# adrianalbert/domain-transfer-GAN

Measured on AMD Instinct MI355X. Metric: training images/sec, 256x256 Augmented CycleGAN step, 1/2/4/8 MI355X, higher is better.
Workload: dtype f32 tensors; conv products as 3 bf16 MFMAs on hi/lo-split fp32 operands (~2^-17 operand rounding), fp32 accumulate; parity vs the reference goldens: losses / single-pass images / cycle reconstructions <= 1e-3 on every fixture at step 0 (measured rec_A / rec_B <= 7.9e-4, profiles/r06_rec_errors.txt)

## Files before the change

### domain-transfer-gan_amd/_lib.py

```python
import ctypes
import os

_HERE = os.path.dirname(os.path.abspath(__file__))
LIB_PATH = os.environ.get("ACGAN_HIP_LIB") or os.path.join(_HERE, "libacgan_hip.so")

ACT_NONE, ACT_RELU, ACT_LRELU, ACT_TANH, ACT_SIGMOID = 0, 1, 2, 3, 4
PAD_ZERO, PAD_REFLECT = 0, 1
IMPL_MFMA, IMPL_DIRECT = 0, 1
PREC_F32, PREC_BF16, PREC_BF16X3 = 0, 1, 2
NLL_LAPLACE, NLL_GAUSSIAN = 0, 1

c_int, c_float, c_size_t, c_void_p = ctypes.c_int, ctypes.c_float, ctypes.c_size_t, ctypes.c_void_p


class ConvDesc(ctypes.Structure):
    _fields_ = [(k, c_int) for k in ("N", "Hi", "Wi", "Ci", "Ho", "Wo", "Co", "K", "stride", "pad", "pad_mode", "Cir", "Cor")]


class LatentMlpParams(ctypes.Structure):
    _fields_ = [("w", c_void_p * 4), ("b", c_void_p * 4), ("gamma", c_void_p * 3), ("beta", c_void_p * 3),
                ("run_mean", c_void_p * 3), ("run_var", c_void_p * 3), ("head_act", c_int)]


class LatentMlpGrads(ctypes.Structure):
    _fields_ = [("dw", c_void_p * 4), ("db", c_void_p * 4), ("dgamma", c_void_p * 3), ("dbeta", c_void_p * 3)]


class AdamGroup(ctypes.Structure):
    _fields_ = [("p", c_void_p), ("g", c_void_p), ("m", c_void_p), ("v", c_void_p), ("n", c_size_t), ("sumsq", c_void_p)]


class EmaGroup(ctypes.Structure):
    _fields_ = [("p", c_void_p), ("e", c_void_p), ("n", c_size_t)]


class PackItem(ctypes.Structure):
    _fields_ = [("w", c_void_p), ("wf", c_void_p), ("wb", c_void_p), ("Or", c_int), ("Ir", c_int), ("K", c_int), ("Ci", c_int), ("Co", c_int)]


MAX_SEGMENTS = 96


class Segments(ctypes.Structure):
    _fields_ = [("dst", c_void_p * MAX_SEGMENTS), ("off", c_int * MAX_SEGMENTS), ("len", c_int * MAX_SEGMENTS), ("n", c_int)]


class NormSumsDesc(ctypes.Structure):
    _fields_ = [("x", c_void_p), ("mean", c_void_p), ("rstd", c_void_p), ("gamma", c_void_p), ("beta", c_void_p),
                ("gstride", c_int), ("sign_mask", c_void_p), ("act", c_int), ("part", c_void_p)]


WINDOW_MAX = 64


class WindowPlan(ctypes.Structure):
    _fields_ = [(k, c_int) for k in ("H", "W", "S", "R", "ny", "nx")] + [("oy", c_int * WINDOW_MAX), ("ox", c_int * WINDOW_MAX)]


ADAM_MAX_GROUPS = 8
EMA_MAX_GROUPS = 8
_P = c_void_p
_D = ctypes.POINTER(ConvDesc)
_MP = ctypes.POINTER(LatentMlpParams)
_MG = ctypes.POINTER(LatentMlpGrads)

SIGNATURES = {
    "acg_version": (c_int, []),
    "acg_last_error": (ctypes.c_char_p, []),
    "acg_last_kernel": (ctypes.c_char_p, []),
    "acg_set_conv_impl": (c_int, [c_int]),
    "acg_set_conv_precision": (c_int, [c_int]),
    "acg_minmax_scale_nhwc_to_nchw": (c_int, [_P, _P, c_int, c_int, c_int, c_int, c_int, _P]),
    "acg_nchw_to_nhwc16": (c_int, [_P, _P, c_int, c_int, c_int, c_int, c_int, _P]),
    "acg_nhwc16_to_nchw": (c_int, [_P, _P, c_int, c_int, c_int, c_int, c_int, _P]),
    "acg_concat_channels": (c_int, [_P, c_int, c_int, _P, c_int, c_int, _P, c_int, c_size_t, _P]),
    "acg_split_channels": (c_int, [_P, c_int, _P, c_int, c_int, _P, c_int, c_int, c_size_t, _P]),
    "acg_ncols_pad": (c_int, [c_int]),
    "acg_packed_wf_elems": (c_size_t, [c_int, c_int, c_int]),
    "acg_packed_wb_elems": (c_size_t, [c_int, c_int, c_int]),
    "acg_pack_conv_weight": (c_int, [_P, c_int, c_int, c_int, c_int, c_int, _P, _P, _P]),
    "acg_pad_vector": (c_int, [_P, c_int, _P, c_int, _P]),
    "acg_conv2d_fwd": (c_int, [_D, _P, _P, _P, _P, c_int, _P]),
    "acg_conv2d_bwd_data_workspace_bytes": (c_size_t, [_D]),
    "acg_conv2d_bwd_data": (c_int, [_D, _P, _P, _P, _P, c_size_t, _P]),
    "acg_s16_encode": (c_int, [_P, _P, c_size_t, _P]),
    "acg_s16_decode": (c_int, [_P, _P, c_size_t, _P]),
    "acg_conv2d_s16_supported": (c_int, [_D]),
    "acg_conv2d_fwd_s16": (c_int, [_D, _P, _P, _P, _P, c_int, _P, c_int, _P]),
    "acg_conv2d_bwd_data_s16": (c_int, [_D, _P, _P, _P, _P, c_size_t, _P, _P, _P, c_int, _P]),
    "acg_conv2d_fwd_s16_mask": (c_int, [_D, _P, _P, _P, _P, _P, _P]),
    "acg_conv2d_bwd_data_s16_mask": (c_int, [_D, _P, _P, _P, _P, c_size_t, _P, _P]),
    "acg_conv2d_bwd_data_s16_sums_supported": (c_int, [_D]),
    "acg_conv2d_bwd_data_s16_sums": (c_int, [_D, _P, _P, _P, _P, c_size_t, _P, _P, ctypes.POINTER(NormSumsDesc), _P]),
    "acg_conv2d_bwd_data_sums_supported": (c_int, [_D]),
    "acg_conv2d_bwd_data_sums": (c_int, [_D, _P, _P, _P, _P, c_size_t, ctypes.POINTER(NormSumsDesc), _P]),
    "acg_conv2d_bwd_weight_s16": (c_int, [_D, _P, _P, _P, _P, c_int, c_int, _P, c_size_t, c_int, _P]),
    "acg_conv2d_bwd_weight_workspace_bytes": (c_size_t, [_D]),
    "acg_conv2d_bwd_weight": (c_int, [_D, _P, _P, _P, _P, c_int, c_int, _P, c_size_t, c_int, _P]),
    "acg_conv_transpose2d_fwd": (c_int, [_D, _P, _P, _P, _P, c_int, _P]),
    "acg_conv_transpose2d_fwd_stats_supported": (c_int, [_D]),
    "acg_conv_transpose2d_fwd_stats": (c_int, [_D, _P, _P, _P, _P, _P, _P]),
    "acg_conv_transpose2d_bwd_data": (c_int, [_D, _P, _P, _P, _P]),
    "acg_conv_transpose2d_bwd_weight": (c_int, [_D, _P, _P, _P, _P, c_int, c_int, _P, c_size_t, c_int, _P]),
    "acg_norm_workspace_bytes": (c_size_t, [c_int, c_size_t, c_int]),
    "acg_conv2d_fwd_stats_supported": (c_int, [_P]),
    "acg_conv2d_bwd_data_add_supported": (c_int, [_P]),
    "acg_conv2d_bwd_data_add": (c_int, [_P, _P, _P, _P, _P, _P, _P, c_size_t, _P]),
    "acg_pack_conv_weights_multi_supported": (c_int, [c_int, c_int, c_int]),
    "acg_pack_conv_weights_multi": (c_int, [_P, c_int, _P]),
    "acg_debug_mid_event": (c_int, [_P]),
    "acg_probe_mfma_rate": (c_int, [_P, c_size_t, c_int, ctypes.POINTER(ctypes.c_double), _P]),
    "acg_mask_apply": (c_int, [_P, _P, _P, c_size_t, _P]),
    "acg_dropout_apply": (c_int, [_P, _P, c_float, _P, c_size_t, _P]),
    "acg_conv2d_bwd_data_relu": (c_int, [_P, _P, _P, _P, _P, _P, c_size_t, _P]),
    "acg_conv2d_fwd_stats": (c_int, [_P, _P, _P, _P, _P, _P, _P]),
    "acg_norm_stats_from_partials": (c_int, [_P, c_int, c_size_t, c_int, c_int, c_float, c_int, _P, _P, _P]),
    "acg_norm_stats": (c_int, [_P, c_int, c_size_t, c_int, c_float, c_int, _P, _P, _P, _P, c_float, _P, c_size_t, _P]),
    "acg_bn_eval_stats": (c_int, [_P, _P, c_int, c_int, c_float, _P, _P, _P]),
    "acg_norm_apply": (c_int, [_P, _P, _P, _P, _P, c_int, _P, _P, _P, c_int, c_size_t, c_int, c_int, c_int, _P]),
    "acg_norm_bwd": (c_int, [_P, _P, _P, _P, _P, _P, _P, _P, c_int, _P, _P, _P, _P, c_int, c_int, c_int, c_size_t, c_int, c_int,
                             c_int, c_int, _P, c_size_t, _P]),
    "acg_norm_bwd_partials": (c_int, [_P, _P, _P, _P, _P, _P, _P, _P, c_int, _P, _P, _P, _P, c_int, c_int, c_int, c_size_t, c_int,
                                      c_int, c_int, c_int, _P, c_int, _P, c_size_t, _P]),
    "acg_norm_bwd_sums": (c_int, [_P, _P, _P, _P, _P, _P, c_int, c_size_t, c_int, c_int, _P, c_size_t, _P]),
    "acg_norm_bwd_apply": (c_int, [_P, _P, _P, _P, _P, _P, c_int, _P, _P, _P, c_int, c_size_t, c_size_t, c_int, c_int, c_int, _P]),
    "acg_act_bwd": (c_int, [_P, _P, _P, c_size_t, c_int, _P]),
    "acg_linear_fwd": (c_int, [_P, _P, _P, _P, c_int, c_int, c_int, c_int, c_int, c_int, _P]),
    "acg_linear_bwd": (c_int, [_P, _P, _P, _P, _P, _P, _P, c_int, c_int, c_int, c_int, c_int, c_int, _P]),
    "acg_latent_mlp_supported": (c_int, [c_int, c_int, c_int]),
    "acg_latent_mlp_fwd": (c_int, [_MP, _P, c_int, c_int, c_int, c_int, c_float, c_float, _P, _P, _P, _P]),
    "acg_latent_mlp_bwd": (c_int, [_MP, _MG, _P, c_int, c_int, c_int, c_int, _P, _P, _P, _P, _P, c_int, _P]),
    "acg_segments_accumulate": (c_int, [_P, ctypes.POINTER(Segments), c_int, _P]),
    "acg_spatial_mean_fwd": (c_int, [_P, _P, c_int, c_size_t, c_int, _P]),
    "acg_spatial_mean_bwd": (c_int, [_P, _P, c_int, c_size_t, c_int, _P]),
    "acg_reduce_workspace_bytes": (c_size_t, [c_size_t]),
    "acg_mse_const_fwd": (c_int, [_P, c_size_t, c_int, c_int, c_float, _P, _P, c_size_t, _P]),
    "acg_mse_const_bwd": (c_int, [_P, c_size_t, c_int, c_int, c_float, _P, _P, _P]),
    "acg_bce_const_fwd": (c_int, [_P, c_size_t, c_int, c_int, c_float, _P, _P, c_size_t, _P]),
    "acg_bce_const_bwd": (c_int, [_P, c_size_t, c_int, c_int, c_float, _P, _P, _P]),
    "acg_l1_fwd": (c_int, [_P, _P, c_size_t, c_int, c_int, _P, _P, c_size_t, _P]),
    "acg_l1_bwd": (c_int, [_P, _P, c_size_t, c_int, c_int, _P, _P, _P, _P]),
    "acg_mean_fwd": (c_int, [_P, c_size_t, c_int, c_int, _P, _P, c_size_t, _P]),
    "acg_sumsq": (c_int, [_P, c_size_t, _P, _P, c_size_t, _P]),
    "acg_pixel_nll_workspace_bytes": (c_size_t, [c_int, c_size_t]),
    "acg_pixel_nll_fwd": (c_int, [c_int, _P, _P, _P, c_int, c_size_t, c_int, c_int, _P, _P, c_size_t, _P]),
    "acg_pixel_nll_bwd": (c_int, [c_int, _P, _P, _P, c_int, c_size_t, c_int, c_int, _P, _P, _P, _P]),
    "acg_latent_bound_step": (c_int, [c_int, c_int, c_int, _P, _P, _P, _P, _P, _P, _P, c_float, c_float, c_float, _P, _P, _P,
                                      _P]),
    "acg_ensemble_workspace_bytes": (c_size_t, [c_int, c_size_t]),
    "acg_ensemble_stats": (c_int, [_P, _P, c_int, c_int, c_size_t, c_int, c_int, ctypes.POINTER(c_float), c_int, _P, _P, _P, _P,
                                   _P, _P, _P, c_size_t, _P]),
    "acg_radial_spectrum_workspace_bytes": (c_size_t, [c_int, c_int, c_int]),
# ... 88 lines not shown
```

### domain-transfer-gan_amd/csrc/conv_internal.h

```cpp
#pragma once
#include "common.h"

#define ACG_KC 16

struct Taps {
    int n;
    short dy[64];
    short dx[64];
    short w[64];
    int pk[64];
    int gpk[64];
    int ngrp;
};

static inline Taps acg_taps_pack(const Taps &t)
{
    Taps r = t;
    for (int i = 0; i < 64; ++i)
        r.pk[i] = i < t.n ? ((t.dy[i] & 0xff) | ((t.dx[i] & 0xff) << 8) | ((int)t.w[i] << 16)) : 0;
    return r;
}

struct Geom {
    int Hin, Win, Cin;
    int Hout, Wout, Cout;
    int GH, GW;
    int os, oy0, ox0;
    int is;
    int reflect;
    int act;
    int ncols_pad;
    long long w_elems;
    int fold_p = 0, fold_H = 0, fold_W = 0;
    float *out2 = nullptr;
    const float *addend = nullptr;
    const unsigned *addend_mask = nullptr;
    const float *relu_src = nullptr;
    int out_s16 = 0, relu_s16 = 0;
    unsigned *mask_out = nullptr;
    const unsigned *relu_mask = nullptr;
    int unpad = 0;
    const float *colfix = nullptr;
    const float *ns_x = nullptr, *ns_mean = nullptr, *ns_rstd = nullptr, *ns_gamma = nullptr, *ns_beta = nullptr;
    const unsigned *ns_mask = nullptr;
    float *ns_part = nullptr;
    int ns_gstride = 0, ns_act = 0;
    float *stats = nullptr;
    int stats_cpi = 0, stats_chunk0 = 0;
    int nphase = 0;
    int ph_ntaps = 0;
    int thin;
    int bk8;
    long long Mtot;
};

int acg_igemm_launch(const float *in, const float *wp, const float *bias, float *out, const Geom &g, const Taps &t,
                     hipStream_t st);

struct WGeom {
    int Hin, Win, Cin;
    int Hg, Wg, Cg;
    int is;
    int reflect;
    int CiP, CoP;
    int nsplit;
    long long Mtot;
    long long m_per_split;
    int thin;
    int bias_from;
    float *bias_part;
};
int acg_wgrad_launch(const float *x, const float *dy, float *part, const WGeom &g, const Taps &t, hipStream_t st);
void acg_wgrad_tiles(int Ci, int Co, int *bci, int *bco, int ntaps);
int acg_wgrad_taps_per_wg(int Ci, int Co, int ntaps, int thin);
bool acg_wgrad_krowg_shape_ok(int K, int stride, int pad, int reflect, int Wi, int Wo, int Cx, int Cg);
bool acg_wgrad_krowg_ok(const WGeom &g, const Taps &t);
int acg_wgrad_krowg_launch(const float *x, const float *dy, float *part, const WGeom &g, const Taps &t, hipStream_t st);

extern int g_acg_precision;
extern int g_acg_conv_impl;

static inline bool use_bf16() { return g_acg_precision != ACG_PREC_F32 && g_acg_conv_impl == ACG_IMPL_MFMA; }
static inline bool bf16x3_mfma() { return g_acg_precision == ACG_PREC_BF16X3 && g_acg_conv_impl == ACG_IMPL_MFMA; }
static inline bool thin_ok(int creal, int K) { return creal >= 1 && creal <= 4 && K > 1 && g_acg_conv_impl == ACG_IMPL_MFMA; }
static inline bool thin_in(const acg_conv_desc *d) { return thin_ok(d->Cir, d->K) && !thin_ok(d->Cor, d->K); }
static inline bool thin_out(const acg_conv_desc *d) { return thin_ok(d->Cor, d->K) && !thin_ok(d->Cir, d->K); }
static inline bool thin_valu_c(int C) { return !use_bf16() && (C == 16 || C == 32 || C == 64); }
__host__ __device__ static inline int c16(int c) { return (c + 15) / 16 * 16; }
__host__ __device__ static inline int wb_slabs(int K) { return K * K + (K == 3 ? 3 : 0); }
enum { ACG_TAIL_NONE = 0, ACG_TAIL_NPACK, ACG_TAIL_TROW };
static inline int pack_tail(int K, int Ck, int Cn)
{
    if (K <= 1 || K > 7) return ACG_TAIL_NONE;
    return c16(Cn) == 16 && c16(Ck) == 32 ? ACG_TAIL_NPACK : (c16(Ck) == 16 && c16(Cn) == 32 ? ACG_TAIL_TROW : ACG_TAIL_NONE);
}
static inline size_t pack_tail_elems(int tail, int K)
{
    return tail == ACG_TAIL_NPACK ? (size_t)K * (K + 3) * 512 : (tail == ACG_TAIL_TROW ? (size_t)K * 1024 : 0);
}
static inline size_t wf_regular_elems(int K, int Ci, int Co) { return (size_t)K * K * (c16(Ci) / 8) * acg_ncols_pad(c16(Co)) * 8; }
static inline size_t wb_regular_elems(int K, int Ci, int Co) { return (size_t)wb_slabs(K) * (c16(Co) / 8) * acg_ncols_pad(c16(Ci)) * 8; }
int acg_igemm_x3_ws_launch(const float *in, const void *wp, const float *bias, float *out, const Geom &g, const Taps &t,
                           long long n_w_elems, hipStream_t st, float *stats = nullptr);
bool acg_igemm_uses_ws(const Geom &g);
bool acg_igemm_x3_pre_ok(const Geom &g, const Taps &t);
int acg_igemm_x3_pre_launch(const void *in, const void *wp, const float *bias, float *out, const Geom &g, const Taps &t,
                            long long n_w_elems, hipStream_t st, float *stats = nullptr);
bool acg_conv_patch16_ok(const Geom &g, const Taps &t);
int acg_conv_patch16_launch(const float *in, const void *wp, const float *bias, float *out, const Geom &g, const Taps &t,
                            long long n_w_elems, hipStream_t st);
bool acg_conv_rows_ok(const Geom &g, const Taps &t);
int acg_conv_rows_launch(const float *in, const void *wp, const float *bias, float *out, const Geom &g, const Taps &t,
                         long long n_w_elems, hipStream_t st);
bool acg_conv_patchn_ok(const Geom &g, const Taps &t);
int acg_conv_patchn_launch(const float *in, const void *wn, const float *bias, float *out, const Geom &g, const Taps &t, hipStream_t st);
bool acg_conv_thinrow_ok(const Geom &g, const Taps &t);
int acg_conv_thinrow_launch(const float *in, const void *wr, const float *bias, float *out, const Geom &g, const Taps &t, hipStream_t st);
bool acg_igemm_ph4_ok(const Geom &g);
bool acg_ph4_plan(const Taps &t, const int nt[4], Taps *out);
int acg_igemm_ph4_launch(const float *in, const void *wp, const float *bias, float *out, const Geom &g, const Taps &plan,
                         long long n_w_elems, hipStream_t st);
int acg_igemm_bf16_launch(const float *in, const void *wp, const float *bias, float *out, const Geom &g, const Taps &t,
                          int bn, long long n_w_elems, hipStream_t st);
int acg_wgrad_bf16_launch(const float *x, const float *dy, float *part, const WGeom &g, const Taps &t, int bci, int bco,
                          hipStream_t st);
bool acg_wgrad_krow_shape_ok(int K, int stride, int pad, int Hi, int Wi, int Ho, int Wo, int Cx, int Cg);
bool acg_wgrad_krow_ok(const WGeom &g, const Taps &t);
int acg_wgrad_krow_launch(const float *x, const float *dy, float *part, const WGeom &g, hipStream_t st);
int acg_wgrad_krow_s16_launch(const void *x, const void *dy, float *part, const WGeom &g, hipStream_t st);
bool acg_wgrad_krow_s_shape_ok(int K, int stride, int pad, int Hi, int Wi, int Ho, int Wo, int Cx, int Cg);
bool acg_wgrad_krow_s_ok(const WGeom &g, const Taps &t);
bool acg_wgrad_thin_patch_shape_ok(int K, int stride, int Hthin, int Wthin, int Hwide, int Wwide, int Cthin, int Cwide);
bool acg_wgrad_thin_patch_ok(const WGeom &g, const Taps &t, int *K, int *flip);
int acg_wgrad_thin_patch_tiles(const WGeom &g);
int acg_wgrad_thin_patch_launch(const float *thin, const float *wide, float *part, const WGeom &g, const Taps &t, hipStream_t st);
int acg_wgrad_krow_s_launch(const float *x, const float *dy, float *part, const WGeom &g, hipStream_t st);

int acg_thin_out_launch(const float *in, const float *wn, const float *bias, float *out, const Geom &g, const Taps &t, hipStream_t st);
int acg_dgrad_colfix_launch(const acg_conv_desc *d, const void *dy, const float *wb, long long w_lo_elems, float *colfix, hipStream_t st);
int acg_reflect_fold_launch(const acg_conv_desc *d, const float *dxp, float *dx, hipStream_t st);
int acg_reflect_fold_frame_launch(const acg_conv_desc *d, const float *dxp, float *dx, const float *addend, const float *relu_src,
                                  const unsigned *addend_mask, int out_s16, int relu_s16, hipStream_t st);
size_t acg_colsum_ws_bytes(long long M, int C);
int acg_colsum_launch(const float *dy, long long M, int C, int Cr, float *db, float *ws, hipStream_t st, int accumulate);
int acg_wgrad_reduce_launch(const float *part, int nsplit, int KK, int CiP, int CoP, int Or, int Ir, float *dw, int thin,
                            int accumulate, const float *bias_part, int Cp, int Cr, float *db, int bias_slots, hipStream_t st);
int acg_direct_fwd_launch(const acg_conv_desc *d, const float *x, const float *wf, const float *bias, float *y, int act, hipStream_t st);
int acg_direct_dgrad_launch(const acg_conv_desc *d, const float *dy, const float *wb, const float *bias, float *dx, int act, hipStream_t st);
int acg_direct_wgrad_launch(const acg_conv_desc *d, const float *x, const float *dy, float *dw, int Or, int Ir, int accumulate, hipStream_t st);

#ifdef __HIPCC__
typedef unsigned acg_u32x4 __attribute__((ext_vector_type(4)));
__device__ __forceinline__ unsigned acg_masked_off(unsigned off, bool ok)
{
    const unsigned keep = 0u - (unsigned)ok;
    return (off & keep) | ~keep;
}
__device__ __forceinline__ void acg_split8(const float (&v)[8], acg_u32x4 &hi, acg_u32x4 &lo)
{
    typedef __bf16 bf16x2_t __attribute__((ext_vector_type(2)));
    typedef float f32x2_t __attribute__((ext_vector_type(2)));
#pragma unroll
    for (int q = 0; q < 4; ++q) {
        const unsigned h = __builtin_bit_cast(unsigned, __builtin_convertvector((f32x2_t){v[2 * q], v[2 * q + 1]}, bf16x2_t));
        const float ha = __builtin_bit_cast(float, h << 16), hb = __builtin_bit_cast(float, h & 0xffff0000u);
        hi[q] = h;
        lo[q] = __builtin_bit_cast(unsigned, __builtin_convertvector((f32x2_t){v[2 * q] - ha, v[2 * q + 1] - hb}, bf16x2_t));
    }
}
__device__ __forceinline__ acg_u32x4 acg_round8(const float (&v)[8])
{
    typedef __bf16 bf16x2_t __attribute__((ext_vector_type(2)));
    typedef float f32x2_t __attribute__((ext_vector_type(2)));
    acg_u32x4 r;
#pragma unroll
    for (int q = 0; q < 4; ++q)
        r[q] = __builtin_bit_cast(unsigned, __builtin_convertvector((f32x2_t){v[2 * q], v[2 * q + 1]}, bf16x2_t));
    return r;
}
#endif
```

### domain-transfer-gan_amd/csrc/conv_x3_pre.hip

```cpp
#include "common.h"
#include "conv_internal.h"
#include <cstdlib>
#include <type_traits>

typedef __bf16 bf16x8 __attribute__((ext_vector_type(8)));
typedef float f32x4 __attribute__((ext_vector_type(4)));
typedef unsigned u32x4 __attribute__((ext_vector_type(4)));

namespace {
constexpr int BM = 128, BN = 128, KC = 32, NK8 = KC / 8;
constexpr int BPL = BN * 8;
constexpr int B_IMG = NK8 * BPL;
__device__ __forceinline__ int lds_at(int plane, int row, int pl) { return plane * pl + ((row ^ (2 * plane)) * 8); }
constexpr int PROW = 80;
constexpr int PPIECES = 11;
constexpr int PIMG = PPIECES * 1024;
constexpr int ABUF = 2 * PIMG;
constexpr int A_BYTES = 2 * ABUF;
constexpr int BBUF = 2 * B_IMG * 2;
constexpr int LDS_BYTES = A_BYTES + 2 * BBUF;
constexpr int NPW = 6;
constexpr unsigned NO_PIX = 0xFFFFFFFFu;
}

// ... 457 lines not shown
                sq += dlt * dlt;
            }
        }
        __syncthreads();
        if (sw) redf[h * BN + c] = sq;
        __syncthreads();
        if (sw && h == 0 && n0 + c < g.Cout) {
            float *o = stats + ((m0 / BM) * 2) * g.Cout + n0 + c;
            o[0] = mu;
            o[g.Cout] = redf[c] + redf[BN + c];
        }
    }
    char *const base0 = (char *)out, *const base1 = (char *)g.out2;
    if (g.out_s16) {
        const char *rsrc = (const char *)g.relu_src;
        constexpr int NK = BM * (BN / 8) / ET;
        u32x4 sv[NK];
#pragma unroll
        for (int k = 0; k < NK; ++k) {
            const int idx = tid + ET * k, row = idx / (BN / 8), c8 = idx - row * (BN / 8);
            const unsigned po = pix_off[row];
            const bool live = po != NO_PIX && (po >> 31) && n0 + c8 * 8 < g.Cout;
            const size_t boff = (size_t)(po & 0x7fffffffu) * 16 + (size_t)(n0 + c8 * 8) * 4;
            if (g.relu_mask != nullptr) sv[k][0] = live ? g.relu_mask[boff >> 7] : 0u;
            else sv[k] = *(const u32x4 *)(rsrc != nullptr && live ? rsrc + boff : in);
        }
#pragma unroll
        for (int k = 0; k < NK; ++k) {
            const int idx = tid + ET * k, row = idx / (BN / 8), c8 = idx - row * (BN / 8);
            const unsigned po = pix_off[row];
            const bool live = po != NO_PIX && n0 + c8 * 8 < g.Cout;
            const size_t boff = (size_t)(po & 0x7fffffffu) * 16 + (size_t)(n0 + c8 * 8) * 4;
            const f32x4 t0 = *(const f32x4 *)&tile[row * TS + c8 * 8], t1 = *(const f32x4 *)&tile[row * TS + c8 * 8 + 4];
            float v[8] = {t0[0], t0[1], t0[2], t0[3], t1[0], t1[1], t1[2], t1[3]};
            if (g.relu_mask != nullptr && (po >> 31)) {
                const unsigned bits = sv[k][0] >> (8 * (c8 & 3));
#pragma unroll
                for (int q = 0; q < 8; ++q) v[q] = (bits >> q) & 1u ? v[q] : 0.f;
            } else if (rsrc != nullptr && (po >> 31)) {
#pragma unroll
                for (int q = 0; q < 4; ++q) {
                    const unsigned a = sv[k][q] & 0xffffu, b = sv[k][q] >> 16;
                    v[2 * q] = (a - 1u) < 0x7fffu ? v[2 * q] : 0.f;
                    v[2 * q + 1] = (b - 1u) < 0x7fffu ? v[2 * q + 1] : 0.f;
                }
            }
            if (g.mask_out != nullptr) {
                unsigned w = 0u;
#pragma unroll
                for (int q = 0; q < 8; ++q) w |= (v[q] > 0.f ? 1u : 0u) << q;
                w = live ? w << (8 * (c8 & 3)) : 0u;
                w |= __shfl_xor(w, 1);
                w |= __shfl_xor(w, 2);
                if (live && (c8 & 3) == 0) g.mask_out[boff >> 7] = w;
            }
            if (!live) continue;
            if (g.fold_p > 0 && !(po >> 31)) {
                *(f32x4 *)(base0 + boff) = t0;
                *(f32x4 *)(base0 + boff + 16) = t1;
                continue;
            }
            acg_u32x4 hi, lo;
            acg_split8(v, hi, lo);
            char *dst = ((po >> 31) ? base1 : base0) + boff;
            *(acg_u32x4 *)dst = hi;
            *(acg_u32x4 *)(dst + 16) = lo;
        }
        TILE_STAMP_END()
        return;
    }
    {
#pragma unroll 4
        for (int k = 0; k < BM * (BN / 4) / ET; ++k) {
            const int idx = tid + ET * k, row = idx / (BN / 4), c4 = idx - row * (BN / 4);
            const unsigned po = pix_off[row];
            if (po != NO_PIX && n0 + c4 * 4 < g.Cout)
                *(f32x4 *)(((po >> 31) ? base1 : base0) + (size_t)(po & 0x7fffffffu) * 16 + (size_t)(n0 + c4 * 4) * 4) = *(const f32x4 *)&tile[row * TS + c4 * 4];
        }
    }
    TILE_STAMP_END()
}
#undef TILE_STAMP_END

static bool pre_rowp(const Geom &g, const Taps &t, int *kdim, int *dxmin, int *kstep)
{
    if (g.is != 1 || g.os != 1 || g.oy0 != 0 || g.ox0 != 0 || g.Hout != g.GH || g.Wout != g.GW) return false;
    int k = 1;
    while (k * k < t.n) ++k;
    if (k * k != t.n || k < 2) return false;
    const int nseg_max = 2 + BM / g.GW, rows_max = BM + nseg_max * (k - 1);
    if (rows_max * 5 > PPIECES * 64 || (BM + (k - 1)) * 5 <= (PPIECES - 1) * 64) return false;
    int mn = t.dx[0];
    for (int i = 1; i < t.n; ++i) mn = t.dx[i] < mn ? t.dx[i] : mn;
    for (int i = 0; i < t.n; ++i)
        if (t.dy[i] != t.dy[(i / k) * k] || t.dx[i] < mn || t.dx[i] >= mn + k) return false;
    const int ks = t.dx[0] == mn ? 1 : -1;
    for (int i = 0; i < t.n; ++i)
        if (t.dx[i] != (ks > 0 ? mn + i % k : mn + k - 1 - i % k)) return false;
    *kdim = k; *dxmin = mn; *kstep = ks;
    return true;
}

bool acg_igemm_x3_pre_ok(const Geom &g, const Taps &t)
{
    int a, b, c;
    return g_acg_precision == ACG_PREC_BF16X3 && g_acg_conv_impl == ACG_IMPL_MFMA && !g.thin && g.Cout >= 128 && g.Cin % 32 == 0 &&
           pre_rowp(g, t, &a, &b, &c);
}

int acg_igemm_x3_pre_launch(const void *in, const void *wp, const float *bias, float *out, const Geom &g0, const Taps &t,
                            long long n_w_elems, hipStream_t st, float *stats)
{
    Geom g = g0;
    g.thin = 0;
    int kdim = 0, dxmin = 0, kstep = 1;
    ACG_REQUIRE(acg_igemm_x3_pre_ok(g, t) && pre_rowp(g, t, &kdim, &dxmin, &kstep), "igemm_conv_x3_pre: unsupported geometry");
    dim3 grid(acg_cdiv(g.Mtot, BM) * (g.ncols_pad / BN));
    const long long nimg = g.Mtot / ((long long)g.GH * g.GW);
    const long long in_bytes = nimg * g.Hin * g.Win * g.Cin * 4;
    const long long out_bytes = nimg * g.Hout * g.Wout * g.Cout * 4;
    const long long w_bytes = n_w_elems * 2 * 2;
    ACG_REQUIRE(in_bytes < (1LL << 32) && w_bytes < (1LL << 32) && out_bytes < (1LL << 34) && g.Mtot < (1LL << 30),
                "igemm_conv_x3_pre: operand exceeds the buffer-addressing limit");
    ACG_REQUIRE(stats == nullptr || (((long long)g.GH * g.GW) % BM == 0 && g.act == ACG_ACT_NONE && !g.out_s16),
                "igemm_conv_x3_pre: per-tile statistics need whole 128-pixel tiles per image, no activation, fp32 output");
    ACG_REQUIRE(!g.out_s16 || (g.addend == nullptr && g.Cout % 8 == 0), "igemm_conv_x3_pre: pre-split output takes no addend");
    ACG_REQUIRE(g.relu_src == nullptr || ((g.fold_p > 0 || g.unpad) && g.out_s16), "igemm_conv_x3_pre: the ReLU source needs the frame path and pre-split output");
    ACG_REQUIRE((g.mask_out == nullptr && g.relu_mask == nullptr) || (g.out_s16 && g.Cout % 32 == 0 && g.ncols_pad == g.Cout && g.fold_p == 0 &&
                                                                        (g.relu_mask == nullptr || (g.unpad && g.relu_src == nullptr))),
                "igemm_conv_x3_pre: sign bitmasks go with pre-split output, 32-multiple channels and the un-padded grid");
    ACG_REQUIRE((g.ns_part == nullptr && (g.addend == nullptr || g.out_s16)) || out_bytes < (1LL << 32),
                "igemm_conv_x3_pre: side inputs (skip addend / norm sums) on a tensor of 4 GiB or more");
    ACG_REQUIRE(g.ns_part == nullptr || (g.unpad && !g.out_s16 && g.Cout % 4 == 0 && (g.ns_act == ACG_ACT_NONE || g.ns_act == ACG_ACT_RELU) &&
                                       g.ns_x != nullptr && g.ns_mean != nullptr && g.ns_rstd != nullptr &&
                                       (g.ns_act == ACG_ACT_NONE || g.ns_mask != nullptr || (g.ns_gamma != nullptr && g.ns_beta != nullptr))),
                "igemm_conv_x3_pre: the norm sums ride on the un-padded fp32 data gradient (act NONE / RELU)");
    ACG_REQUIRE(!g.unpad || (g.GW % BM == 0 && g.GH >= 4 && kdim == 3 && !g.reflect && g.fold_p == 0 && g.out2 == out && g.act == ACG_ACT_NONE),
                "igemm_conv_x3_pre: the un-padded reflect data gradient needs whole-row tiles of a 3x3 layer");
    const unsigned inb = (unsigned)in_bytes, wb = (unsigned)w_bytes, wlo = (unsigned)(n_w_elems * 2);
    const Taps tp = acg_taps_pack(t);
#define X3_PRE(R, S, U) hipLaunchKernelGGL((igemm_conv_x3_pre<R, S, U>), grid, dim3(512), 0, st, (const char *)in, (const __bf16 *)wp, bias, out, g, tp, inb, wb, wlo, stats, kdim, dxmin, kstep)
    ACG_REQUIRE(g.ns_part == nullptr || (!g.reflect && stats == nullptr), "igemm_conv_x3_pre: norm sums on a forward launch");
    if (g.reflect) { if (stats) X3_PRE(true, true, false); else X3_PRE(true, false, false); }
    else if (g.ns_part != nullptr) X3_PRE(false, false, true);
    else { if (stats) X3_PRE(false, true, false); else X3_PRE(false, false, false); }
#undef X3_PRE
    ACG_CHECK_LAUNCH("igemm_conv_x3_pre");
    acg_note_kernel("igemm_conv_x3_pre<REFLECT=%d,STATS=%d%s>", g.reflect ? 1 : 0, stats ? 1 : 0, g.ns_part != nullptr ? ",SUMS=1" : "");
    return ACG_OK;
}
```

### include/acgan_hip.h

```cpp
#ifndef ACGAN_HIP_H
#define ACGAN_HIP_H

#include <stddef.h>
#include <stdint.h>

#ifdef __cplusplus
extern "C" {
#endif

#define ACG_VERSION 118

typedef enum {
    ACG_OK = 0,
    ACG_ERR_INVALID = -1,
    ACG_ERR_WORKSPACE = -2,
    ACG_ERR_LAUNCH = -3,
    ACG_ERR_COMM = -4
} acg_status;

typedef enum {
    ACG_ACT_NONE = 0, ACG_ACT_RELU = 1, ACG_ACT_LRELU = 2 , ACG_ACT_TANH = 3, ACG_ACT_SIGMOID = 4
} acg_act;
typedef enum { ACG_PAD_ZERO = 0, ACG_PAD_REFLECT = 1 } acg_pad_mode;
typedef enum { ACG_IMPL_MFMA = 0, ACG_IMPL_DIRECT = 1 } acg_conv_impl;
typedef enum { ACG_PREC_F32 = 0, ACG_PREC_BF16 = 1, ACG_PREC_BF16X3 = 2 } acg_precision;

typedef struct {
    int N, Hi, Wi, Ci;
    int Ho, Wo, Co;
    int K, stride, pad, pad_mode;
    int Cir, Cor;
} acg_conv_desc;

int acg_version(void);
const char *acg_last_error(void);
const char *acg_last_kernel(void);
int acg_debug_mid_event(void *event);
int acg_probe_mfma_rate(float *scratch, size_t scratch_floats, int iters, double *flops_out, void *stream);
int acg_set_conv_impl(int impl);
int acg_set_conv_precision(int prec);

int acg_minmax_scale_nhwc_to_nchw(const float *raw, float *out_nchw, int N, int H, int W, int Craw, int C, void *stream);

int acg_nchw_to_nhwc16(const float *src, float *dst, int N, int C, int H, int W, int Cp, void *stream);
int acg_nhwc16_to_nchw(const float *src, float *dst, int N, int C, int H, int W, int Cp, void *stream);
int acg_concat_channels(const float *a, int Ca, int Cap, const float *b, int Cb, int Cbp, float *dst, int Cdp,
                        size_t npix, void *stream);
int acg_split_channels(const float *gdst, int Cdp, float *ga, int Ca, int Cap, float *gb, int Cb, int Cbp,
                       size_t npix, void *stream);

int acg_ncols_pad(int c);
size_t acg_packed_wf_elems(int K, int Ci, int Co);
size_t acg_packed_wb_elems(int K, int Ci, int Co);
int acg_pack_conv_weight(const float *w_oihw, int Or, int Ir, int K, int Ci, int Co, float *wf, float *wb, void *stream);
typedef struct {
    const float *w;
    float *wf, *wb;
    int Or, Ir, K, Ci, Co;
} acg_pack_item;
int acg_pack_conv_weights_multi_supported(int Or, int Ir, int K);
int acg_pack_conv_weights_multi(const acg_pack_item *items, int n, void *stream);
int acg_pad_vector(const float *src, int n, float *dst, int np, void *stream);

int acg_conv2d_fwd(const acg_conv_desc *d, const float *x, const float *wf, const float *bias, float *y, int act,
                   void *stream);
int acg_conv2d_fwd_stats_supported(const acg_conv_desc *d);
int acg_conv2d_fwd_stats(const acg_conv_desc *d, const float *x, const float *wf, const float *bias, float *y,
                         float *stats, void *stream);
size_t acg_conv2d_bwd_data_workspace_bytes(const acg_conv_desc *d);
int acg_conv2d_bwd_data(const acg_conv_desc *d, const float *dy, const float *wb, float *dx, void *workspace,
                        size_t ws_bytes, void *stream);
int acg_conv2d_bwd_data_add_supported(const acg_conv_desc *d);
int acg_conv2d_bwd_data_add(const acg_conv_desc *d, const float *dy, const float *wb, const float *addend,
                            const unsigned *addend_sign_mask, float *dx, void *ws, size_t ws_bytes, void *stream);
int acg_conv2d_bwd_data_relu(const acg_conv_desc *d, const float *dy, const float *wb, const float *x, float *dx,
                             void *ws, size_t ws_bytes, void *stream);
int acg_s16_encode(const float *x, void *y_s16, size_t n, void *stream);
int acg_s16_decode(const void *x_s16, float *y, size_t n, void *stream);
int acg_conv2d_s16_supported(const acg_conv_desc *d);
int acg_conv2d_fwd_s16(const acg_conv_desc *d, const void *x_s16, const float *wf, const float *bias, void *y, int act,
                       float *stats, int out_s16, void *stream);
int acg_conv2d_bwd_data_s16(const acg_conv_desc *d, const void *dy_s16, const float *wb, void *dx, void *ws, size_t ws_bytes,
                            const float *addend, const unsigned *addend_sign_mask, const void *relu_src_s16, int out_s16,
                            void *stream);
typedef struct acg_norm_sums {
    const float *x, *mean, *rstd;
    const float *gamma, *beta;
    int gstride;
    const unsigned *sign_mask;
    int act;
    float *part;
} acg_norm_sums;
int acg_conv2d_bwd_data_s16_sums_supported(const acg_conv_desc *d);
int acg_conv2d_bwd_data_s16_sums(const acg_conv_desc *d, const void *dy_s16, const float *wb, float *dx, void *ws,
                                 size_t ws_bytes, const float *addend, const unsigned *addend_sign_mask,
                                 const acg_norm_sums *ns, void *stream);
int acg_conv2d_bwd_data_sums_supported(const acg_conv_desc *d);
int acg_conv2d_bwd_data_sums(const acg_conv_desc *d, const float *dy, const float *wb, float *dx, void *ws, size_t ws_bytes,
                             const acg_norm_sums *ns, void *stream);
int acg_conv2d_fwd_s16_mask(const acg_conv_desc *d, const void *x_s16, const float *wf, const float *bias, void *y_s16,
                            unsigned *sign_mask, void *stream);
int acg_conv2d_bwd_data_s16_mask(const acg_conv_desc *d, const void *dy_s16, const float *wb, void *dx_s16, void *ws,
                                 size_t ws_bytes, const unsigned *relu_sign_mask, void *stream);
int acg_conv2d_bwd_weight_s16(const acg_conv_desc *d, const void *x_s16, const void *dy_s16, float *dw, float *db, int Or,
                              int Ir, void *ws, size_t ws_bytes, int accumulate, void *stream);
size_t acg_conv2d_bwd_weight_workspace_bytes(const acg_conv_desc *d);
int acg_conv2d_bwd_weight(const acg_conv_desc *d, const float *x, const float *dy, float *dw_oihw, float *db,
                          int Or, int Ir, void *workspace, size_t ws_bytes, int accumulate, void *stream);

int acg_conv_transpose2d_fwd(const acg_conv_desc *d, const float *x, const float *wb, const float *bias, float *y,
                             int act, void *stream);
int acg_conv_transpose2d_fwd_stats_supported(const acg_conv_desc *d);
int acg_conv_transpose2d_fwd_stats(const acg_conv_desc *d, const float *x, const float *wb, const float *bias, float *y,
                                   float *stats, void *stream);
int acg_conv_transpose2d_bwd_data(const acg_conv_desc *d, const float *dy, const float *wf, float *dx, void *stream);
int acg_conv_transpose2d_bwd_weight(const acg_conv_desc *d, const float *x, const float *dy, float *dw_oihw,
                                    float *db, int Or, int Ir, void *workspace, size_t ws_bytes, int accumulate,
                                    void *stream);

// ... 191 lines not shown
```

Measured before the change: 222.4.

## Add 256-pixel tile bf16x3 conv kernel with dedicated DMA producer waves

Adds a new implicit-GEMM conv kernel for 3x3 reflect-padded layers with 128-multiple channels. It uses a 256x128 output tile, 768 threads (8 MFMA waves plus 4 producer waves issuing buffer-to-LDS loads), and 4-deep weight buffering. The aim is to raise weight and patch reuse per workgroup and to overlap the loads with the MFMA work. The existing 128-pixel kernel now dispatches to it when the geometry qualifies. The cost is a larger LDS footprint and lower occupancy (3 waves/EU), plus fewer workgroups on smaller layers, which could hurt load balance.

Measured after the change: 224.1, median of 6. About the same (+0.7%).

```diff
diff --git a/domain-transfer-gan_amd/_lib.py b/domain-transfer-gan_amd/_lib.py
--- a/domain-transfer-gan_amd/_lib.py
+++ b/domain-transfer-gan_amd/_lib.py
@@ -68,6 +68,7 @@
     "acg_version": (c_int, []),
     "acg_last_error": (ctypes.c_char_p, []),
     "acg_last_kernel": (ctypes.c_char_p, []),
+    "acg_last_x3_tile_pixels": (c_int, []),
     "acg_set_conv_impl": (c_int, [c_int]),
     "acg_set_conv_precision": (c_int, [c_int]),
     "acg_minmax_scale_nhwc_to_nchw": (c_int, [_P, _P, c_int, c_int, c_int, c_int, c_int, _P]),
diff --git a/domain-transfer-gan_amd/csrc/conv_internal.h b/domain-transfer-gan_amd/csrc/conv_internal.h
--- a/domain-transfer-gan_amd/csrc/conv_internal.h
+++ b/domain-transfer-gan_amd/csrc/conv_internal.h
@@ -106,6 +106,11 @@
 bool acg_igemm_x3_pre_ok(const Geom &g, const Taps &t);
 int acg_igemm_x3_pre_launch(const void *in, const void *wp, const float *bias, float *out, const Geom &g, const Taps &t,
                             long long n_w_elems, hipStream_t st, float *stats = nullptr);
+bool acg_x3_pre_rowp(const Geom &g, const Taps &t, int *kdim, int *dxmin, int *kstep);
+bool acg_igemm_x3_t256_ok(const Geom &g, const Taps &t);
+int acg_igemm_x3_t256_launch(const void *in, const void *wp, const float *bias, float *out, const Geom &g, const Taps &t,
+                             long long n_w_elems, hipStream_t st, float *stats);
+void acg_note_x3_tile(int pixels);
 bool acg_conv_patch16_ok(const Geom &g, const Taps &t);
 int acg_conv_patch16_launch(const float *in, const void *wp, const float *bias, float *out, const Geom &g, const Taps &t,
                             long long n_w_elems, hipStream_t st);
diff --git a/domain-transfer-gan_amd/csrc/conv_x3_pre.hip b/domain-transfer-gan_amd/csrc/conv_x3_pre.hip
--- a/domain-transfer-gan_amd/csrc/conv_x3_pre.hip
+++ b/domain-transfer-gan_amd/csrc/conv_x3_pre.hip
@@ -563,7 +563,7 @@
 }
 #undef TILE_STAMP_END
 
-static bool pre_rowp(const Geom &g, const Taps &t, int *kdim, int *dxmin, int *kstep)
+bool acg_x3_pre_rowp(const Geom &g, const Taps &t, int *kdim, int *dxmin, int *kstep)
 {
     if (g.is != 1 || g.os != 1 || g.oy0 != 0 || g.ox0 != 0 || g.Hout != g.GH || g.Wout != g.GW) return false;
     int k = 1;
@@ -586,7 +586,7 @@
 {
     int a, b, c;
     return g_acg_precision == ACG_PREC_BF16X3 && g_acg_conv_impl == ACG_IMPL_MFMA && !g.thin && g.Cout >= 128 && g.Cin % 32 == 0 &&
-           pre_rowp(g, t, &a, &b, &c);
+           acg_x3_pre_rowp(g, t, &a, &b, &c);
 }
 
 int acg_igemm_x3_pre_launch(const void *in, const void *wp, const float *bias, float *out, const Geom &g0, const Taps &t,
@@ -595,7 +595,12 @@
     Geom g = g0;
     g.thin = 0;
     int kdim = 0, dxmin = 0, kstep = 1;
-    ACG_REQUIRE(acg_igemm_x3_pre_ok(g, t) && pre_rowp(g, t, &kdim, &dxmin, &kstep), "igemm_conv_x3_pre: unsupported geometry");
+    ACG_REQUIRE(acg_igemm_x3_pre_ok(g, t) && acg_x3_pre_rowp(g, t, &kdim, &dxmin, &kstep), "igemm_conv_x3_pre: unsupported geometry");
+    if (acg_igemm_x3_t256_ok(g, t)) {
+        if (int rc = acg_igemm_x3_t256_launch(in, wp, bias, out, g, t, n_w_elems, st, stats)) return rc;
+        acg_note_kernel("igemm_conv_x3_pre<REFLECT=1,STATS=%d>", stats ? 1 : 0);
+        return ACG_OK;
+    }
     dim3 grid(acg_cdiv(g.Mtot, BM) * (g.ncols_pad / BN));
     const long long nimg = g.Mtot / ((long long)g.GH * g.GW);
     const long long in_bytes = nimg * g.Hin * g.Win * g.Cin * 4;
@@ -627,6 +632,7 @@
     else { if (stats) X3_PRE(false, true, false); else X3_PRE(false, false, false); }
 #undef X3_PRE
     ACG_CHECK_LAUNCH("igemm_conv_x3_pre");
+    acg_note_x3_tile(BM);
     acg_note_kernel("igemm_conv_x3_pre<REFLECT=%d,STATS=%d%s>", g.reflect ? 1 : 0, stats ? 1 : 0, g.ns_part != nullptr ? ",SUMS=1" : "");
     return ACG_OK;
 }
diff --git a/domain-transfer-gan_amd/csrc/conv_x3_t256.hip b/domain-transfer-gan_amd/csrc/conv_x3_t256.hip
--- /dev/null
+++ b/domain-transfer-gan_amd/csrc/conv_x3_t256.hip
@@ -0,0 +1,403 @@
+#include "common.h"
+#include "conv_internal.h"
+#include <type_traits>
+
+typedef __bf16 bf16x8 __attribute__((ext_vector_type(8)));
+typedef float f32x4 __attribute__((ext_vector_type(4)));
+typedef unsigned u32x4 __attribute__((ext_vector_type(4)));
+
+namespace {
+constexpr int BM = 256, BN = 128, KC = 32, NK8 = KC / 8;
+constexpr int BPL = BN * 8;
+constexpr int B_IMG = NK8 * BPL;
+__device__ __forceinline__ int lds_at(int plane, int row, int pl) { return plane * pl + ((row ^ (2 * plane)) * 8); }
+constexpr int PROW = 80;
+constexpr int PPIECES = 21;
+constexpr int PIMG = PPIECES * 1024;
+constexpr int ABUF = 2 * PIMG;
+constexpr int A_BYTES = 2 * ABUF;
+constexpr int BBUF = 2 * B_IMG * 2;
+constexpr int NBUF = 4;
+constexpr int LDS_BYTES = A_BYTES + NBUF * BBUF;
+constexpr int NPW = 11;
+constexpr int NT = 768;
+constexpr int NB_PIECES = 4;
+constexpr unsigned NO_PIX = 0xFFFFFFFFu;
+static_assert(PIMG % 256 == 0 && (BM + 2 * 2) * 5 <= PPIECES * 64 && (BM + 2) * 5 > (PPIECES - 1) * 64, "patch piece plan");
+static_assert(LDS_BYTES + 3072 <= 160 * 1024, "LDS");
+#ifdef T256_ABL_NO_WEIGHT_DMA
+constexpr bool W_ON = false;
+#else
+constexpr bool W_ON = true;
+#endif
+#ifdef T256_ABL_NO_PATCH_DMA
+constexpr bool A_ON = false;
+#else
+constexpr bool A_ON = true;
+#endif
+#ifdef T256_ABL_NO_EPILOGUE_TRAFFIC
+constexpr bool E_ON = false;
+#else
+constexpr bool E_ON = true;
+#endif
+int s_last_tile = 0;
+}
+
+void acg_note_x3_tile(int pixels) { s_last_tile = pixels; }
+extern "C" int acg_last_x3_tile_pixels(void) { return s_last_tile; }
+
+template <bool STATS>
+__global__ __launch_bounds__(NT) __attribute__((amdgpu_waves_per_eu(3, 3))) void
+igemm_conv_x3_t256(const char *__restrict__ in, const __bf16 *__restrict__ wp, const float *__restrict__ bias,
+                   float *__restrict__ out, Geom g, Taps taps, unsigned in_bytes, unsigned w_bytes, unsigned w_lo_bytes,
+                   float *__restrict__ stats, int dxmin)
+{
+    __shared__ __attribute__((aligned(1024))) char lds[LDS_BYTES + BM * 4 + 2 * 2 * BN * 4];
+    unsigned *const pix_off = (unsigned *)(lds + LDS_BYTES);
+    float *const red = (float *)(lds + LDS_BYTES + BM * 4);
+
+    const int tid = threadIdx.x, lane = tid & 63, wave = __builtin_amdgcn_readfirstlane(tid >> 6);
+    const int nwg = gridDim.x, bid = blockIdx.x;
+    const int xq = nwg >> 3, xr = nwg & 7, xcd = bid & 7;
+    const int swz = (xcd < xr ? xcd * (xq + 1) : xr * (xq + 1) + (xcd - xr) * xq) + (bid >> 3);
+    const int tiles_n = g.ncols_pad / BN;
+    const int tile_n = swz % tiles_n, tile_m = swz / tiles_n;
+    const int n0 = tile_n * BN;
+    const int m0 = tile_m * BM;
+    const int Mt = (int)g.Mtot;
+    const int S = taps.n * (g.Cin / KC);
+
+    const int grow0 = m0 / g.GW;
+    const int x0 = m0 - grow0 * g.GW;
+    const int first = g.GW - x0 < BM ? g.GW - x0 : BM;
+    const int img = grow0 / g.GH, gy0 = grow0 - img * g.GH;
+
+    typedef __attribute__((address_space(3))) void lds_void;
+    if (wave >= 8) {
+        const int pt = tid - 512, pw = wave - 8;
+        constexpr int BCH = NK8 * BN, BL = BCH / 256;
+        static_assert(2 * BL == NB_PIECES, "the vmcnt plan counts 2 * BL B pieces per stage");
+        const __amdgpu_buffer_rsrc_t rin = __builtin_amdgcn_make_buffer_rsrc((void *)in, 0, in_bytes, 0x00020000);
+        const __amdgpu_buffer_rsrc_t rw = __builtin_amdgcn_make_buffer_rsrc((void *)wp, 0, w_bytes, 0x00020000);
+        unsigned b_voff[BL];
+        int b_lds[BL];
+#pragma unroll
+        for (int i = 0; i < BL; ++i) {
+            const int idx = pt + 256 * i;
+            const int plane = idx / BN, slot = idx - plane * BN, col = slot ^ (2 * plane);
+            b_voff[i] = (unsigned)((((plane >> 1) * g.ncols_pad + n0 + col) * 16 + (plane & 1) * 8) * 2);
+            b_lds[i] = __builtin_amdgcn_readfirstlane((plane * BPL + (slot & ~63) * 8) * 2);
+        }
+        const int tap_v = taps.pk[lane < taps.n ? lane : 0];
+        auto tap_pk = [&](int t) { return __builtin_amdgcn_readlane(tap_v, t); };
+        int bt = 0, bc0 = 0, bs = 0;
+        auto dma_b = [&]() {
+            if (W_ON || bs < NBUF) {
+                char *Bb = lds + A_BYTES + (bs & (NBUF - 1)) * BBUF;
+                const int slab = tap_pk(bt) >> 16;
+                const unsigned soff = (unsigned)(((slab * (g.Cin >> 4) + (bc0 >> 4)) * g.ncols_pad) * 16) * 2u;
+#pragma unroll
+                for (int i = 0; i < BL; ++i) {
+                    __builtin_amdgcn_raw_ptr_buffer_load_lds(rw, (lds_void *)(Bb + b_lds[i]), 16, b_voff[i], soff, 0, 0);
+                    __builtin_amdgcn_raw_ptr_buffer_load_lds(rw, (lds_void *)(Bb + B_IMG * 2 + b_lds[i]), 16, b_voff[i], soff + w_lo_bytes, 0, 0);
+                }
+            }
+            ++bs;
+            if (++bt == taps.n) { bt = 0; bc0 += KC; }
+        };
+        dma_b();
+        dma_b();
+        dma_b();
+        dma_b();
+
+        const int nrows = BM + (first >= BM ? 1 : 2) * 2;
+        int pa_gy[NPW], pa_nb[NPW], pa_lds[NPW];
+        unsigned pa_col[NPW];
+        bool pa_ok[NPW];
+#pragma unroll
+        for (int j = 0; j < NPW; ++j) {
+            const int e = pw + 4 * j;
+            const int q = e >= PPIECES ? 1 : 0, pc = e - q * PPIECES;
+            const int L = pc * 64 + lane;
+            const int row = L / 5, ch = L - row * 5;
+            const int seg = row >= first + 2 ? 1 : 0, px = row - seg * (first + 2);
+            int ix = (seg == 0 ? x0 : 0) + px + dxmin;
+            ix = ix < 0 ? -ix : ix;
+            ix = ix >= g.Win ? 2 * (g.Win - 1) - ix : ix;
+            pa_gy[j] = gy0 + seg;
+            pa_nb[j] = img * g.Hin;
+            pa_col[j] = (unsigned)(ix * g.Cin * 4 + (q + 2 * (ch >> 1)) * 32 + (ch & 1) * 16);
+            pa_ok[j] = e < 2 * PPIECES && ch < 4 && row < nrows;
+            pa_lds[j] = __builtin_amdgcn_readfirstlane(q * PIMG + pc * 1024);
+        }
+        const int nA = pw < 2 ? NPW : NPW - 1;
+        constexpr int NPW0 = 6;
+        int ar_t = 0, ar_c0 = 0, ar_row = 0;
+        auto dma_a = [&](auto part_c) {
+            constexpr int PART = decltype(part_c)::value;
+            if (A_ON || ar_row < 2) {
+                const int ty = (tap_pk(ar_t) << 24) >> 24;
+                char *Ab = lds + (ar_row & 1) * ABUF;
+#pragma unroll
+                for (int j = PART == 0 ? 0 : NPW0; j < (PART == 0 ? NPW0 : NPW); ++j) {
+                    if (pw + 4 * j < 2 * PPIECES) {
+                        int iy = pa_gy[j] + ty;
+                        iy = iy < 0 ? -iy : iy;
+                        iy = iy >= g.Hin ? 2 * (g.Hin - 1) - iy : iy;
+                        const unsigned off = (unsigned)((pa_nb[j] + iy) * g.Win) * (unsigned)(g.Cin * 4) + pa_col[j] + (unsigned)(ar_c0 * 4);
+                        __builtin_amdgcn_raw_ptr_buffer_load_lds(rin, (lds_void *)(Ab + pa_lds[j]), 16, acg_masked_off(off, pa_ok[j]), 0, 0, 0);
+                    }
+                }
+            }
+            if (PART == 0) return;
+            ++ar_row;
+            ar_t += 3;
+            if (ar_t >= taps.n) { ar_t = 0; ar_c0 += KC; }
+        };
+        const std::integral_constant<int, 0> part0{};
+        const std::integral_constant<int, 1> part1{};
+        auto bundle_n = [&](int s, int ph) {
+            const int nb = (W_ON || s < NBUF) ? NB_PIECES : 0;
+            if (s == 0) return nb + nA;
+            if (ph == 2) return nb + ((A_ON || (s + 1) / 3 < 2) ? NPW0 : 0);
+            if (ph == 0) return nb + ((A_ON || s / 3 < 2) ? nA - NPW0 : 0);
+            return nb;
+        };
+        auto wait_vm = [](auto nc) {
+            constexpr int N = decltype(nc)::value;
+            asm volatile("" ::: "memory");
+            __builtin_amdgcn_s_waitcnt(0x0F70 | (N & 15) | ((N >> 4) << 14));
+            asm volatile("" ::: "memory");
+        };
+        auto wait_left = [&](int n) {
+            if (n >= 2 * NB_PIECES + NPW) wait_vm(std::integral_constant<int, 2 * NB_PIECES + NPW>{});
+            else if (n >= 2 * NB_PIECES + NPW - 1) wait_vm(std::integral_constant<int, 2 * NB_PIECES + NPW - 1>{});
+            else if (n >= NB_PIECES + NPW0) wait_vm(std::integral_constant<int, NB_PIECES + NPW0>{});
+            else if (n >= NB_PIECES + NPW - NPW0) wait_vm(std::integral_constant<int, NB_PIECES + NPW - NPW0>{});
+            else if (n >= NB_PIECES + NPW - NPW0 - 1) wait_vm(std::integral_constant<int, NB_PIECES + NPW - NPW0 - 1>{});
+            else if (n >= NB_PIECES) wait_vm(std::integral_constant<int, NB_PIECES>{});
+            else wait_vm(std::integral_constant<int, 0>{});
+        };
+        dma_a(part0);
+        dma_a(part1);
+        dma_a(part0);
+        dma_a(part1);
+        {
+            const int seg = pt >= first ? 1 : 0, gx = seg ? pt - first : x0 + pt;
+            pix_off[pt] = m0 + pt < Mt ? (unsigned)(((((long long)img * g.Hout + gy0 + seg) * g.Wout + gx) * g.Cout) >> 2) : NO_PIX;
+        }
+        wait_left(nA);
+        __builtin_amdgcn_s_barrier();
+        int ph = 0;
+        for (int s = 0; s < S; ++s) {
+            wait_left(s == 0 ? 0 : s + 3 < S ? bundle_n(s + 3, ph) : 0);
+            __builtin_amdgcn_s_barrier();
+            if (s + 4 < S) {
+                if (ph == 1) dma_a(part0);
+                if (ph == 2) dma_a(part1);
+                dma_b();
+            }
+            ph = ph == 2 ? 0 : ph + 1;
+        }
+    } else {
+        const int wm = wave >> 1, wn = wave & 1;
+        constexpr int TM = 64, TN = 64;
+        f32x4 acc[4][4];
+        const int pl = lane >> 4, lr = lane & 15;
+        __builtin_amdgcn_s_setprio(2);
+#pragma unroll
+        for (int i = 0; i < 4; ++i)
+#pragma unroll
+            for (int j = 0; j < 4; ++j) acc[i][j] = (f32x4){0.f, 0.f, 0.f, 0.f};
+        int a_base[4];
+        {
+#pragma unroll
+            for (int i = 0; i < 4; ++i) {
+                const int tp = wm * TM + i * 16 + lr;
+                const int arow = tp < first ? tp : tp + 2;
+                a_base[i] = (pl & 1) * PIMG + arow * PROW + (pl >> 1) * 32;
+            }
+        }
+        const int b_base = 2 * lds_at(pl, wn * TN + lr, BPL);
+        const char *ldsb = (const char *)lds;
+        const char *pb0 = ldsb + A_BYTES + b_base;
+        struct AF { bf16x8 h[4], l[4]; };
+        struct BF { bf16x8 h, l; };
+        auto load_a = [&](AF &f, int k, int i) {
+            const char *po = ldsb + ((k / 3) & 1) * ABUF + (k % 3) * PROW;
+            f.h[i] = *(const bf16x8 *)(po + a_base[i]);
+            f.l[i] = *(const bf16x8 *)(po + a_base[i] + 16);
+        };
+        auto load_b = [&](int k, int j) {
+            const char *pb = pb0 + (k & (NBUF - 1)) * BBUF + j * 256;
+            BF f;
+            f.h = *(const bf16x8 *)pb;
+            f.l = *(const bf16x8 *)(pb + 2 * B_IMG);
+            return f;
+        };
+        auto mma = [&](int j, const AF &a, const BF &b) {
+#pragma unroll
+            for (int i = 0; i < 4; ++i) {
+                acc[i][j] = __builtin_amdgcn_mfma_f32_16x16x32_bf16(a.l[i], b.h, acc[i][j], 0, 0, 0);
+                acc[i][j] = __builtin_amdgcn_mfma_f32_16x16x32_bf16(a.h[i], b.l, acc[i][j], 0, 0, 0);
+                acc[i][j] = __builtin_amdgcn_mfma_f32_16x16x32_bf16(a.h[i], b.h, acc[i][j], 0, 0, 0);
+            }
+        };
+        __syncthreads();
+        AF af[2];
+        BF b0, b1;
+#pragma unroll
+        for (int i = 0; i < 4; ++i) load_a(af[0], 0, i);
+        b0 = load_b(0, 0);
+        for (int it = 0; it < S / 12; ++it) {
+#pragma unroll
+            for (int k = 0; k < 12; ++k) {
+                const int kn = (k + 1) % 12;
+                b1 = load_b(k, 1);
+                load_a(af[kn & 1], kn, 0);
+                __builtin_amdgcn_sched_barrier(0);
+                mma(0, af[k & 1], b0);
+                b0 = load_b(k, 2);
+                load_a(af[kn & 1], kn, 1);
+                __builtin_amdgcn_sched_barrier(0);
+                mma(1, af[k & 1], b1);
+                b1 = load_b(k, 3);
+                load_a(af[kn & 1], kn, 2);
+                load_a(af[kn & 1], kn, 3);
+                __builtin_amdgcn_sched_barrier(0);
+                mma(2, af[k & 1], b0);
+                __syncthreads();
+                b0 = load_b(kn, 0);
+                __builtin_amdgcn_sched_barrier(0);
+                mma(3, af[k & 1], b1);
+                __builtin_amdgcn_sched_barrier(0);
+            }
+        }
+        __builtin_amdgcn_s_setprio(0);
+        __syncthreads();
+        float *tile = (float *)lds;
+#pragma unroll
+        for (int j = 0; j < 4; ++j) {
+            const int cl = wn * TN + j * 16 + lr;
+            const float bv = (bias != nullptr && n0 + cl < g.Cout) ? bias[n0 + cl] : 0.f;
+#pragma unroll
+            for (int i = 0; i < 4; ++i)
+#pragma unroll
+                for (int r = 0; r < 4; ++r)
+                    tile[(wm * TM + i * 16 + 4 * pl + r) * BN + cl] = acg_apply_act(acc[i][j][r] + bv, STATS ? (int)ACG_ACT_NONE : g.act);
+        }
+    }
+    constexpr int TS = BN;
+    static_assert(BM * TS * 4 <= LDS_BYTES, "the staged tile must fit the LDS buffers");
+    float *tile = (float *)lds;
+    if (wave >= 8) __syncthreads();
+    __syncthreads();
+    if constexpr (STATS) {
+        const int ck = tid >> 8, c = tid & (BN - 1), h = (tid >> 7) & 1;
+        const bool sw = tid < 512;
+        float *redf = red + (ck & 1) * 2 * BN;
+        const float *tc = tile + (ck & 1) * 128 * TS;
+        float sum = 0.f;
+        if (sw) {
+#pragma unroll 8
+            for (int r = 0; r < 64; ++r) sum += tc[(h * 64 + r) * TS + c];
+            redf[h * BN + c] = sum;
+        }
+        __syncthreads();
+        const float mu = (redf[c] + redf[BN + c]) * (1.f / 128);
+        float sq = 0.f;
+        if (sw) {
+#pragma unroll 8
+            for (int r = 0; r < 64; ++r) {
+                const float dlt = tc[(h * 64 + r) * TS + c] - mu;
+                sq += dlt * dlt;
+            }
+        }
+        __syncthreads();
+        if (sw) redf[h * BN + c] = sq;
+        __syncthreads();
+        if (sw && h == 0 && n0 + c < g.Cout) {
+            float *o = stats + ((size_t)(m0 / 128 + ck) * 2) * g.Cout + n0 + c;
+            o[0] = mu;
+            o[g.Cout] = redf[c] + redf[BN + c];
+        }
+    }
+    if (!E_ON) return;
+    char *const base0 = (char *)out;
+    if (g.out_s16) {
+        constexpr int NITEM = BM * (BN / 8), NK = (NITEM + NT - 1) / NT;
+#pragma unroll
+        for (int k = 0; k < NK; ++k) {
+            const int idx = tid + NT * k;
+            const bool in_tile = idx < NITEM;
+            const int row = in_tile ? idx / (BN / 8) : 0, c8 = idx & (BN / 8 - 1);
+            const unsigned po = pix_off[row];
+            const bool live = in_tile && po != NO_PIX && n0 + c8 * 8 < g.Cout;
+            const size_t boff = (size_t)po * 16 + (size_t)(n0 + c8 * 8) * 4;
+            const f32x4 t0 = *(const f32x4 *)&tile[row * TS + c8 * 8], t1 = *(const f32x4 *)&tile[row * TS + c8 * 8 + 4];
+            float v[8] = {t0[0], t0[1], t0[2], t0[3], t1[0], t1[1], t1[2], t1[3]};
+            if (g.mask_out != nullptr) {
+                unsigned w = 0u;
+#pragma unroll
+                for (int q = 0; q < 8; ++q) w |= (v[q] > 0.f ? 1u : 0u) << q;
+                w = live ? w << (8 * (c8 & 3)) : 0u;
+                w |= __shfl_xor(w, 1);
+                w |= __shfl_xor(w, 2);
+                if (live && (c8 & 3) == 0) g.mask_out[boff >> 7] = w;
+            }
+            if (!live) continue;
+            acg_u32x4 hi, lo;
+            acg_split8(v, hi, lo);
+            char *dst = base0 + boff;
+            *(acg_u32x4 *)dst = hi;
+            *(acg_u32x4 *)(dst + 16) = lo;
+        }
+        return;
+    }
+    {
+        constexpr int NITEM = BM * (BN / 4), NK = (NITEM + NT - 1) / NT;
+#pragma unroll 4
+        for (int k = 0; k < NK; ++k) {
+            const int idx = tid + NT * k, row = idx / (BN / 4), c4 = idx - row * (BN / 4);
+            if (idx >= NITEM) break;
+            const unsigned po = pix_off[row];
+            if (po != NO_PIX && n0 + c4 * 4 < g.Cout)
+                *(f32x4 *)(base0 + (size_t)po * 16 + (size_t)(n0 + c4 * 4) * 4) = *(const f32x4 *)&tile[row * TS + c4 * 4];
+        }
+    }
+}
+
+bool acg_igemm_x3_t256_ok(const Geom &g, const Taps &t)
+{
+    int k = 0, dxmin = 0, ks = 0;
+    return acg_igemm_x3_pre_ok(g, t) && acg_x3_pre_rowp(g, t, &k, &dxmin, &ks) && k == 3 && ks == 1 && g.reflect && !g.unpad &&
+           g.fold_p == 0 && g.addend == nullptr && g.relu_src == nullptr && g.relu_mask == nullptr && g.ns_part == nullptr &&
+           g.colfix == nullptr && g.Cin % 128 == 0 && g.Cout % 128 == 0 && g.ncols_pad == g.Cout &&
+           ((long long)g.GH * g.GW) % BM == 0 && (g.GW == 128 || g.GW % BM == 0) && g.Win == g.GW && g.Hin == g.GH;
+}
+
+int acg_igemm_x3_t256_launch(const void *in, const void *wp, const float *bias, float *out, const Geom &g, const Taps &t,
+                             long long n_w_elems, hipStream_t st, float *stats)
+{
+    int kdim = 0, dxmin = 0, kstep = 1;
+    ACG_REQUIRE(acg_igemm_x3_t256_ok(g, t) && acg_x3_pre_rowp(g, t, &kdim, &dxmin, &kstep), "igemm_conv_x3_t256: unsupported geometry");
+    dim3 grid((unsigned)(g.Mtot / BM) * (g.ncols_pad / BN));
+    const long long nimg = g.Mtot / ((long long)g.GH * g.GW);
+    const long long in_bytes = nimg * g.Hin * g.Win * g.Cin * 4;
+    const long long out_bytes = nimg * g.Hout * g.Wout * g.Cout * 4;
+    const long long w_bytes = n_w_elems * 2 * 2;
+    ACG_REQUIRE(in_bytes < (1LL << 32) && w_bytes < (1LL << 32) && out_bytes < (1LL << 34) && g.Mtot < (1LL << 30),
+                "igemm_conv_x3_t256: operand exceeds the buffer-addressing limit");
+    ACG_REQUIRE(stats == nullptr || (g.act == ACG_ACT_NONE && !g.out_s16),
+                "igemm_conv_x3_t256: per-tile statistics need no activation and fp32 output");
+    ACG_REQUIRE(!g.out_s16 || g.Cout % 8 == 0, "igemm_conv_x3_t256: pre-split output needs 8-multiple channels");
+    ACG_REQUIRE(g.mask_out == nullptr || (g.out_s16 && g.Cout % 32 == 0), "igemm_conv_x3_t256: the sign bitmask goes with pre-split output");
+    const unsigned inb = (unsigned)in_bytes, wb = (unsigned)w_bytes, wlo = (unsigned)(n_w_elems * 2);
+    const Taps tp = acg_taps_pack(t);
+#define X3_T256(S) hipLaunchKernelGGL((igemm_conv_x3_t256<S>), grid, dim3(NT), 0, st, (const char *)in, (const __bf16 *)wp, bias, out, g, tp, inb, wb, wlo, stats, dxmin)
+    if (stats) X3_T256(true); else X3_T256(false);
+#undef X3_T256
+    ACG_CHECK_LAUNCH("igemm_conv_x3_t256");
+    acg_note_x3_tile(BM);
+    return ACG_OK;
+}
diff --git a/include/acgan_hip.h b/include/acgan_hip.h
--- a/include/acgan_hip.h
+++ b/include/acgan_hip.h
@@ -35,6 +35,7 @@
 int acg_version(void);
 const char *acg_last_error(void);
 const char *acg_last_kernel(void);
+int acg_last_x3_tile_pixels(void);
 int acg_debug_mid_event(void *event);
 int acg_probe_mfma_rate(float *scratch, size_t scratch_floats, int iters, double *flops_out, void *stream);
 int acg_set_conv_impl(int impl);
```
